# zzz5y/street_crafter

Measured on AMD Instinct MI355X. Metric: frames/sec @1M Gaussians 1920x1280 + PSNR vs ref; 1/2/4/8 MI355X, higher is better.
Workload: dtype f32

## Files before the change

### include/street_crafter_amd.h

```cpp
#ifndef STREET_CRAFTER_AMD_H
#define STREET_CRAFTER_AMD_H

#include <stddef.h>
#include <stdint.h>

#ifdef __cplusplus
extern "C" {
#endif

typedef void* sc_stream_t;

#define SC_OK 0
#define SC_EINVAL (-1)
#define SC_EWORKSPACE (-2)
#define SC_EUNSUPPORTED (-3)

const char* sc_version(void);
const char* sc_error_string(int code);
const char* sc_target_arch(void);
int sc_wait_i64(const int64_t* addr, int64_t value, int64_t timeout_us);

int sc_projection_fwd(const float* means, const float* quats, const float* scales,
                      const float* viewmats, const float* Ks, int C, int N, int width, int height,
                      float eps2d, float near_plane, float far_plane, float radius_clip,
// ... 33 lines not shown
                       const int32_t* tile_work ,
                       const float* viewmats ,
                       int32_t* view_registry ,
                       int32_t* tile_order ,
                       sc_stream_t stream);
int sc_view_slots(void);
int sc_view_registry_words(void);
int sc_isect_bin_bucket_capacity(void);
int sc_isect_split_limits(int64_t* out );
int64_t sc_isect_split_seg_bound(int64_t n_records, int nsb);
int sc_isect_split_bins(const uint64_t* keys, int64_t n, uint64_t lo, uint64_t hi, int32_t* bins);
int sc_isect_split_plan(const uint32_t* bin_counts, int cap, int32_t* range_of_bin, int32_t* n_ranges);
int sc_isect_bin_sort(const float* means2d, const int32_t* radii, const float* depths, int C, int N,
                      int tile_size, int tile_width, int tile_height,
                      const int32_t* isect_offsets, const int64_t* meta_dev,
                      void* count_workspace ,
                      int64_t capacity, int64_t rec_capacity, int64_t super_capacity,
                      int64_t* isect_ids , int32_t* flatten_ids,
                      void* workspace, size_t ws_bytes, sc_stream_t stream);
int sc_isect_ids_rebuild(const int32_t* flatten_ids, const int32_t* isect_offsets, const float* depths,
                         int C, int N, int tile_width, int tile_height, int64_t n_isects,
                         int64_t* isect_ids, sc_stream_t stream);
int sc_isect_bin_reset_cursors(void* count_workspace, int64_t CN, int C, int tile_width, int tile_height,
                               sc_stream_t stream);

int sc_isect_offsets(const int64_t* isect_ids, int64_t n_isects, int C, int tile_width,
                     int tile_height, int32_t* offsets, sc_stream_t stream);

int sc_sh_fwd(int degree, const float* dirs, const float* coeffs, const uint8_t* masks,
              int64_t M, int K, float* colors, sc_stream_t stream);
int sc_sh_bwd(int degree, const float* dirs, const float* coeffs, const uint8_t* masks,
              int64_t M, int K, const float* v_colors, float* v_coeffs, float* v_dirs,
              sc_stream_t stream);

int sc_rasterize_fwd(const float* means2d, const float* conics, const float* colors,
                     const float* opacities, const float* backgrounds, const uint8_t* tile_masks,
                     int C, int N, int D, int width, int height, int tile_size,
                     int tile_width, int tile_height,
                     const int32_t* isect_offsets, const int32_t* flatten_ids, int64_t n_isects,
                     float* render_colors, float* render_alphas,
                     int32_t* last_ids ,
                     const int32_t* tile_order ,
                     int32_t* tile_work ,
                     sc_stream_t stream);
int sc_tile_order_len(int total_tiles);
int sc_rasterize_bwd(const float* means2d, const float* conics, const float* colors,
                     const float* opacities, const float* backgrounds, const uint8_t* tile_masks,
                     int C, int N, int D, int width, int height, int tile_size,
                     int tile_width, int tile_height,
                     const int32_t* isect_offsets, const int32_t* flatten_ids, int64_t n_isects,
                     const float* render_alphas, const int32_t* last_ids,
                     const float* v_render_colors, const float* v_render_alphas,
                     float* v_means2d_abs, float* v_means2d, float* v_conics, float* v_colors,
                     float* v_opacities, const int32_t* tile_order ,
                     sc_stream_t stream);

size_t sc_knn_workspace_bytes(int64_t n);
int sc_knn3_mean_dist2(const float* points, int64_t n, float* out, void* workspace,
                       size_t ws_bytes, sc_stream_t stream);

int sc_point_project(const float* points, const float* colors, const float* opacities , float occ,
                     const float* radius_in , int N, const double* viewmat, double fx,
                     double fy, double cx, double cy, double focal_r, int width, int height, double near_plane,
                     double far_plane, int radius_mode, double scale, float knn_scale_down, int32_t* radii,
                     float* means2d, float* depths, float* records, sc_stream_t stream);
int sc_point_rasterize_fwd(const float* records, int N, int width, int height, int tile_width, int tile_height,
// ... 322 lines not shown
```

### street_crafter_amd/_lib.py

```python
from __future__ import annotations

import ctypes as C
import os

_HERE = os.path.dirname(os.path.abspath(__file__))
LIB_PATH = os.path.join(_HERE, "lib", "libstreet_crafter_hip.so")
DIAG_LIB_PATH = os.path.join(_HERE, "lib", "libstreet_crafter_hip_diag.so")

_lib = None
_path = LIB_PATH
_lock = __import__("threading").Lock()


def use_diagnostic_build(tag: str = ""):
    global _path
    want = DIAG_LIB_PATH.replace("_diag.so", f"_diag_{tag}.so") if tag else DIAG_LIB_PATH
    if _lib is not None and _path != want:
        raise RuntimeError("use_diagnostic_build() must be called before the library is first loaded")
    if not os.path.exists(want):
        raise ImportError(f"diagnostic library not built ({want} missing): "
                          "python -m street_crafter_amd.build --diag")
    _path = want

c_f32p = C.c_void_p
# ... 60 lines not shown
                                    c_f32p, c_f32p, c_f32p, c_stream]),
    "sc_projection_bwd": (C.c_int, [c_f32p, c_f32p, c_f32p, c_f32p, c_f32p, C.c_int, C.c_int, C.c_int,
                                    C.c_int, C.c_float, c_i32p, c_f32p, c_f32p, c_f32p, c_f32p, c_f32p,
                                    c_f32p, c_f32p, c_f32p, c_f32p, c_stream]),
    "sc_isect_workspace_bytes": (C.c_size_t, [C.c_int64]),
    "sc_isect_count": (C.c_int, [c_f32p, c_i32p, C.c_int, C.c_int, C.c_int, C.c_int, C.c_int, c_i32p,
                                 c_i64p, C.c_void_p, C.c_size_t, c_stream]),
    "sc_isect_emit": (C.c_int, [c_f32p, c_i32p, c_f32p, C.c_int, C.c_int, C.c_int, C.c_int, C.c_int,
                                c_i32p, C.c_int64, c_i64p, c_i32p, C.c_void_p, C.c_size_t, c_stream]),
    "sc_radix_sort_workspace_bytes": (C.c_size_t, [C.c_int64]),
    "sc_radix_sort_pairs_u64_i32": (C.c_int, [c_u64p, c_i32p, c_u64p, c_i32p, C.c_int64, C.c_int,
                                              C.c_void_p, C.c_size_t, c_stream]),
    "sc_isect_bin_workspace_bytes": (C.c_size_t, [C.c_int64, C.c_int, C.c_int, C.c_int, C.c_int64]),
    "sc_isect_bin_count": (C.c_int, [c_f32p, c_i32p, c_f32p, C.c_int, C.c_int, C.c_int, C.c_int, C.c_int, c_i32p,
                                     c_i32p, c_i64p, c_i64p, C.c_int64, C.c_void_p, C.c_size_t, c_i32p, c_f32p, c_i32p,
                                     c_i32p, c_stream]),
    "sc_view_slots": (C.c_int, []),
    "sc_view_registry_words": (C.c_int, []),
    "sc_isect_bin_bucket_capacity": (C.c_int, []),
    "sc_isect_split_limits": (C.c_int, [c_i64p]),
    "sc_isect_split_seg_bound": (C.c_int64, [C.c_int64, C.c_int]),
    "sc_isect_split_bins": (C.c_int, [c_u64p, C.c_int64, C.c_uint64, C.c_uint64, c_i32p]),
    "sc_isect_split_plan": (C.c_int, [C.c_void_p, C.c_int, c_i32p, c_i32p]),
    "sc_isect_bin_sort": (C.c_int, [c_f32p, c_i32p, c_f32p, C.c_int, C.c_int, C.c_int, C.c_int, C.c_int,
                                    c_i32p, c_i64p, C.c_void_p, C.c_int64, C.c_int64, C.c_int64, c_i64p,
                                    c_i32p, C.c_void_p, C.c_size_t, c_stream]),
    "sc_isect_ids_rebuild": (C.c_int, [c_i32p, c_i32p, c_f32p, C.c_int, C.c_int, C.c_int, C.c_int, C.c_int64, c_i64p,
                                       c_stream]),
    "sc_isect_bin_reset_cursors": (C.c_int, [C.c_void_p, C.c_int64, C.c_int, C.c_int, C.c_int, c_stream]),
    "sc_isect_offsets": (C.c_int, [c_i64p, C.c_int64, C.c_int, C.c_int, C.c_int, c_i32p, c_stream]),
    "sc_sh_fwd": (C.c_int, [C.c_int, c_f32p, c_f32p, c_u8p, C.c_int64, C.c_int, c_f32p, c_stream]),
    "sc_sh_bwd": (C.c_int, [C.c_int, c_f32p, c_f32p, c_u8p, C.c_int64, C.c_int, c_f32p, c_f32p, c_f32p,
                            c_stream]),
    "sc_rasterize_fwd": (C.c_int, [c_f32p, c_f32p, c_f32p, c_f32p, c_f32p, c_u8p, C.c_int, C.c_int, C.c_int,
                                   C.c_int, C.c_int, C.c_int, C.c_int, C.c_int, c_i32p, c_i32p, C.c_int64,
                                   c_f32p, c_f32p, c_i32p, c_i32p, c_i32p, c_stream]),
    "sc_rasterize_fwd_ed": (C.c_int, [c_f32p, c_f32p, c_f32p, c_f32p, c_f32p, c_u8p, C.c_int, C.c_int, C.c_int,
                                      C.c_int, C.c_int, C.c_int, C.c_int, C.c_int, c_i32p, c_i32p, C.c_int64,
                                      c_f32p, c_f32p, c_i32p, c_i32p, c_stream]),
    "sc_rasterize_fwd_planar": (C.c_int, [c_f32p, c_f32p, c_f32p, c_f32p, c_f32p, c_u8p, C.c_int, C.c_int, C.c_int,
                                          C.c_int, C.c_int, C.c_int, C.c_int, C.c_int, c_i32p, c_i32p, C.c_int64,
                                          c_f32p, c_f32p, c_i32p, c_i32p, c_stream]),
    "sc_group_extents": (C.c_int, [c_i32p, c_i32p, C.c_int64, c_u8p, C.c_int, C.c_int, C.c_int, C.c_int, C.c_int,
                                   c_i32p, c_stream]),
    "sc_rasterize_fwd_groups": (C.c_int, [c_f32p, c_f32p, c_f32p, c_f32p, c_u8p, c_i32p, C.c_int, C.c_int, C.c_int,
                                          C.c_int, C.c_int, C.c_int, C.c_int, C.c_int, C.c_int, c_i32p, c_i32p,
                                          C.c_int64, c_f32p, c_f32p, c_f32p, c_f32p, c_stream]),
    "sc_rasterize_fwd_groups_ids": (C.c_int, [c_f32p, c_f32p, c_f32p, c_f32p, c_u8p, c_i32p, C.c_int, C.c_int, C.c_int,
                                              C.c_int, C.c_int, C.c_int, C.c_int, C.c_int, C.c_int, c_i32p, c_i32p,
                                              C.c_int64, c_f32p, c_f32p, c_f32p, c_f32p, c_i32p, c_stream]),
    "sc_rasterize_bwd_groups": (C.c_int, [c_f32p, c_f32p, c_f32p, c_f32p, c_u8p, C.c_int, C.c_int, C.c_int, C.c_int,
                                          C.c_int, C.c_int, C.c_int, C.c_int, C.c_int, c_i32p, c_i32p, C.c_int64,
                                          c_f32p, c_f32p, c_i32p, c_f32p, c_f32p, c_f32p, c_f32p, c_f32p, c_f32p,
                                          c_f32p, c_f32p, c_f32p, c_stream]),
    "sc_camera_centers": (C.c_int, [c_f32p, C.c_int, c_f32p, c_stream]),
    "sc_projection_sh_fwd": (C.c_int, [c_f32p, c_f32p, c_f32p, c_f32p, c_f32p, c_f32p, c_f32p, c_f32p,
                                       C.c_int, C.c_int, C.c_int, C.c_int, C.c_int, C.c_int, C.c_float,
                                       C.c_float, C.c_float, C.c_float, C.c_int, c_i32p, c_f32p, c_f32p,
                                       c_f32p, c_f32p, c_f32p, c_f32p, c_stream]),
    "sc_projection_sh_bwd": (C.c_int, [c_f32p, c_f32p, c_f32p, c_f32p, c_f32p, c_f32p, c_f32p, c_f32p,
                                       C.c_int, C.c_int, C.c_int, C.c_int, C.c_int, C.c_int, C.c_float, C.c_int,
                                       c_i32p, c_f32p, c_f32p, c_f32p, c_f32p, c_f32p, c_f32p, c_f32p, c_f32p,
                                       c_f32p, c_f32p, c_f32p, c_stream]),
    "sc_rasterize_fwd_packed": (C.c_int, [c_f32p, c_f32p, c_u8p, C.c_int, C.c_int, C.c_int, C.c_int, C.c_int, C.c_int,
                                          c_i32p, c_i32p, C.c_int64, c_f32p, c_f32p, c_i32p, c_i32p, C.c_int, c_stream]),
    "sc_records_unpack": (C.c_int, [c_f32p, C.c_int64, c_f32p, c_f32p, c_f32p, c_stream]),
# ... 208 lines not shown
```

### street_crafter_amd/build.py

```python
from __future__ import annotations

import concurrent.futures as cf
import os
import subprocess
import sys

HERE = os.path.dirname(os.path.abspath(__file__))
CSRC = os.path.join(HERE, "csrc")
LIBDIR = os.path.join(HERE, "lib")
OBJDIR = os.path.join(HERE, "build")
LIB = os.path.join(LIBDIR, "libstreet_crafter_hip.so")
LIB_DIAG = os.path.join(LIBDIR, "libstreet_crafter_hip_diag.so")
BINDING = os.path.join(LIBDIR, "_sc_fast.so")
ARCH = "gfx950"

SOURCES = ["capi.hip", "projection.hip", "isect.hip", "isect_bin.hip", "radix_sort.hip", "sh.hip",
           "raster_fwd.hip", "raster_probe.hip", "raster_groups.hip", "raster_groups_bwd.hip", "raster_layers.hip", "raster_bwd.hip", "knn.hip", "fused_fwd.hip", "fused_bwd.hip", "point_raster.hip",
           "losses.hip", "regularizers.hip", "optim.hip", "densify.hip", "cubemap.hip", "lpips.hip", "resize.hip", "compose.hip",
           "frame_tail.hip", "point_assemble.hip", "frame_viz.hip"]
COMMON_FLAGS = ["-O3", f"--offload-arch={ARCH}", "-fPIC", "-std=c++17", "-Wall", "-Wno-unused-function",
                "-fno-gpu-rdc"]


def abi_hash() -> str:
    import hashlib
    with open(os.path.join(HERE, "..", "include", "street_crafter_amd.h"), "rb") as f:
        return hashlib.sha256(f.read()).hexdigest()[:16]


def _hipcc():
    for c in (os.environ.get("HIPCC"), "/opt/rocm/bin/hipcc", "hipcc"):
        if c and (os.path.isabs(c) and os.path.exists(c) or not os.path.isabs(c)):
            return c
    raise RuntimeError("hipcc not found")


def _deps(src):
    d = [os.path.join(CSRC, src)]
    d += [os.path.join(CSRC, f) for f in os.listdir(CSRC) if f.endswith(".h")]
    d.append(os.path.join(HERE, "..", "include", "street_crafter_amd.h"))
    return d


def _stale(target, deps):
    if not os.path.exists(target):
        return True
    t = os.path.getmtime(target)
    return any(os.path.getmtime(d) > t for d in deps)


def _compile(src, force, verbose, diag=False):
    tag = os.environ.get("SC_DIAG_TAG", "") if diag else ""
# ... 67 lines not shown
```

### street_crafter_amd/csrc/sh.hip

```cpp
#include "sh_common.h"

#pragma clang fp contract(off)

namespace {

template <int DEG>
__global__ __launch_bounds__(256) void sh_fwd_kernel(const float* __restrict__ dirs,
                                                     const float* __restrict__ coeffs,
                                                     const uint8_t* __restrict__ masks, int64_t M,
                                                     int K, float* __restrict__ colors) {
    const int64_t i = (int64_t)blockIdx.x * 256 + threadIdx.x;
    if (i >= M) return;
    float r = 0.f, g = 0.f, b = 0.f;
    if (!masks || masks[i])
        sh_eval<DEG>(dirs[i * 3 + 0], dirs[i * 3 + 1], dirs[i * 3 + 2], coeffs + i * (int64_t)K * 3, r, g, b);
    colors[i * 3 + 0] = r; colors[i * 3 + 1] = g; colors[i * 3 + 2] = b;
}

}

#pragma clang fp contract(fast)

namespace {

template <int DEG, bool VEC>
__global__ __launch_bounds__(256) void sh_bwd_kernel(const float* __restrict__ dirs,
                                                     const float* __restrict__ coeffs,
                                                     const uint8_t* __restrict__ masks, int64_t M,
                                                     int K, const float* __restrict__ v_colors,
                                                     float* __restrict__ v_coeffs,
                                                     float* __restrict__ v_dirs) {
    constexpr int NB = (DEG + 1) * (DEG + 1);
    constexpr int NV = (NB * 3 + 3) / 4;
    const int64_t i = (int64_t)blockIdx.x * 256 + threadIdx.x;
    if (i >= M) return;
    float* vc = v_coeffs + i * (int64_t)K * 3;
    const bool on = !masks || masks[i];
    float vdx = 0.f, vdy = 0.f, vdz = 0.f;
    if (on) {
        const float dx = dirs[i * 3 + 0], dy = dirs[i * 3 + 1], dz = dirs[i * 3 + 2];
        float Y[NB];
        sh_basis<DEG>(dx, dy, dz, Y);
        const float vr = v_colors[i * 3 + 0], vg = v_colors[i * 3 + 1], vb = v_colors[i * 3 + 2];
        if (VEC) {
            float o[NV * 4];
#pragma unroll
            for (int f = 0; f < NV * 4; ++f) o[f] = (f < NB * 3) ? Y[f / 3] * ((f % 3) == 0 ? vr : ((f % 3) == 1 ? vg : vb)) : 0.f;
// ... 24 lines not shown
                w[k] = VEC ? vr * cf[k * 3 + 0] + vg * cf[k * 3 + 1] + vb * cf[k * 3 + 2]
                           : vr * c[k * 3 + 0] + vg * c[k * 3 + 1] + vb * c[k * 3 + 2];
            sh_dir_vjp<DEG>(dx, dy, dz, w, vdx, vdy, vdz);
        }
    } else if (VEC) {
        for (int j = 0; j < (K * 3) / 4; ++j) reinterpret_cast<float4*>(vc)[j] = make_float4(0.f, 0.f, 0.f, 0.f);
    } else {
        for (int k = 0; k < K; ++k) { vc[k * 3 + 0] = 0.f; vc[k * 3 + 1] = 0.f; vc[k * 3 + 2] = 0.f; }
    }
    if (v_dirs) { v_dirs[i * 3 + 0] = vdx; v_dirs[i * 3 + 1] = vdy; v_dirs[i * 3 + 2] = vdz; }
}

}

extern "C" int sc_sh_fwd(int degree, const float* dirs, const float* coeffs, const uint8_t* masks,
                         int64_t M, int K, float* colors, sc_stream_t stream) {
    if (degree < 0 || degree > 4 || M < 0 || K < (degree + 1) * (degree + 1)) return SC_EINVAL;
    if (M == 0) return SC_OK;
    if (!dirs || !coeffs || !colors) return SC_EINVAL;
    const int64_t nb = (M + 255) / 256;
    if (nb > 0x7fffffff) return SC_EINVAL;
    dim3 grid((unsigned)nb), block(256);
    switch (degree) {
        case 0: hipLaunchKernelGGL(sh_fwd_kernel<0>, grid, block, 0, sc_s(stream), dirs, coeffs, masks, M, K, colors); break;
        case 1: hipLaunchKernelGGL(sh_fwd_kernel<1>, grid, block, 0, sc_s(stream), dirs, coeffs, masks, M, K, colors); break;
        case 2: hipLaunchKernelGGL(sh_fwd_kernel<2>, grid, block, 0, sc_s(stream), dirs, coeffs, masks, M, K, colors); break;
        case 3: hipLaunchKernelGGL(sh_fwd_kernel<3>, grid, block, 0, sc_s(stream), dirs, coeffs, masks, M, K, colors); break;
        default: hipLaunchKernelGGL(sh_fwd_kernel<4>, grid, block, 0, sc_s(stream), dirs, coeffs, masks, M, K, colors); break;
    }
    SC_LAUNCH_CHECK();
    return SC_OK;
}

extern "C" int sc_sh_bwd(int degree, const float* dirs, const float* coeffs, const uint8_t* masks,
                         int64_t M, int K, const float* v_colors, float* v_coeffs, float* v_dirs,
                         sc_stream_t stream) {
    if (degree < 0 || degree > 4 || M < 0 || K < (degree + 1) * (degree + 1)) return SC_EINVAL;
    if (M == 0) return SC_OK;
    if (!dirs || !coeffs || !v_colors || !v_coeffs) return SC_EINVAL;
    const int64_t nb = (M + 255) / 256;
    if (nb > 0x7fffffff) return SC_EINVAL;
    dim3 grid((unsigned)nb), block(256);
    const bool vec = (K * 3) % 4 == 0 && ((uintptr_t)coeffs % 16) == 0 && ((uintptr_t)v_coeffs % 16) == 0;
#define SC_SH_BWD(D)                                                                                              \
    if (vec) hipLaunchKernelGGL((sh_bwd_kernel<D, true>), grid, block, 0, sc_s(stream), dirs, coeffs, masks, M, K, \
                                v_colors, v_coeffs, v_dirs);                                                       \
    else hipLaunchKernelGGL((sh_bwd_kernel<D, false>), grid, block, 0, sc_s(stream), dirs, coeffs, masks, M, K,     \
                            v_colors, v_coeffs, v_dirs)
    switch (degree) {
        case 0: SC_SH_BWD(0); break;
        case 1: SC_SH_BWD(1); break;
        case 2: SC_SH_BWD(2); break;
        case 3: SC_SH_BWD(3); break;
        default: SC_SH_BWD(4); break;
    }
#undef SC_SH_BWD
    SC_LAUNCH_CHECK();
    return SC_OK;
}
```

### street_crafter_amd/dist.py

```python
from __future__ import annotations

import os
import socket
import subprocess
import sys
import time
from typing import Callable, Dict, List, Optional, Sequence

import torch
import torch.distributed as dist

from . import _lib

ROUNDING = {"video": 0, "save_image": 1}


def frames_for_rank(n_frames: int, rank: int, world: int) -> List[int]:
    return list(range(rank, n_frames, world))


def _hwc_view(x: torch.Tensor):
    if x.dim() != 3 or x.shape[0] != 3:
        return None
    s0, s1, s2 = x.stride()
    if s0 == 1 and s2 >= 3 and s1 == x.shape[2] * s2:
        return x, s2, 1
    if s2 == 1 and s1 == x.shape[2] and s0 >= x.shape[1] * x.shape[2]:
        return x, 1, s0
    return None


_STREAM_FN = []


def _raw_stream(t: torch.Tensor):
    if not _STREAM_FN:
        from .rendering import _stream
        _STREAM_FN.append(_stream)
    return _STREAM_FN[0](t)


def to_uint8_frame(rgb_chw: torch.Tensor, acc: Optional[torch.Tensor] = None,
                   sky_rgb_chw: Optional[torch.Tensor] = None, rounding: str = "video",
                   out: Optional[torch.Tensor] = None) -> torch.Tensor:
    if rounding not in ROUNDING:
        raise ValueError(f"rounding must be one of {sorted(ROUNDING)}, got {rounding!r}")
    if (acc is None) != (sky_rgb_chw is None):
        raise ValueError("acc and sky_rgb_chw go together (two-pass frame) or are both None")
    x = rgb_chw.detach() if rgb_chw.requires_grad else rgb_chw
    H, W = x.shape[1], x.shape[2]
    if out is None:
        out = torch.empty((H, W, 3), dtype=torch.uint8, device=x.device)
    else:
        assert out.shape == (H, W, 3) and out.dtype == torch.uint8 and out.is_contiguous() and out.device == x.device
    if x.is_cuda and x.dtype == torch.float32:
        fg = _hwc_view(x)
        sky = _hwc_view(sky_rgb_chw.detach()) if sky_rgb_chw is not None else None
        a = acc.detach().reshape(H, W) if acc is not None else None
        if fg is not None and (sky_rgb_chw is None or (sky is not None and a.is_contiguous()
                                                      and a.dtype == torch.float32)):
            b = _lib.binding()
            if fg[2] != 1 or fg[1] < 3 or (sky is not None and (sky[2] != 1 or sky[1] < 3)):
                rc = b.frame_composite_u8_strided(fg[0].data_ptr(), fg[1], fg[2], 0 if a is None else a.data_ptr(),
                                                  0 if sky is None else sky[0].data_ptr(), 1 if sky is None else sky[1],
                                                  1 if sky is None else sky[2], H * W, ROUNDING[rounding], out,
                                                  _raw_stream(x))
            else:
                rc = b.frame_composite_u8(fg[0].data_ptr(), fg[1], 0 if a is None else a.data_ptr(),
                                          0 if sky is None else sky[0].data_ptr(), 0 if sky is None else sky[1],
                                          H * W, ROUNDING[rounding], out, _raw_stream(x))
            if rc:
                _lib.check(rc, "sc_frame_composite_u8")
            return out
    v = x.float().clamp(0.0, 1.0)
    if sky_rgb_chw is not None:
        v = (v + sky_rgb_chw.detach().float().clamp(0.0, 1.0) * (1.0 - acc.detach().float().reshape(1, H, W))).clamp(0.0, 1.0)
    v = v * 255.0
    if ROUNDING[rounding]:
        v = v + 0.5
    out.copy_(v.to(torch.uint8).permute(1, 2, 0))
    return out
# ... 373 lines not shown
```

### street_crafter_amd/isect.py

```python
from __future__ import annotations

import collections
import math
import os
import threading
import weakref
from typing import Optional, Tuple

import torch
from torch import Tensor

from . import _lib
from .lazy import LazyTensor as _LazyTensor


def _env_on(name: str, default: bool = True) -> bool:
    v = os.environ.get(name)
    return default if v is None or v == "" else v not in ("0", "false", "False", "off", "no")


class _Switches:
    __slots__ = ("tile_order", "lazy_ids", "view_slots", "packed_records", "defer_isect", "planar_out", "fused_train")

    def __init__(self):
        self.tile_order = _env_on("SC_TILE_ORDER")
        self.lazy_ids = _env_on("SC_LAZY_IDS")
        self.view_slots = _env_on("SC_VIEW_SLOTS")
        self.packed_records = _env_on("SC_PACKED_RECORDS")
        self.defer_isect = _env_on("SC_DEFER_ISECT")
        self.planar_out = _env_on("SC_PLANAR_OUTPUT")
        self.fused_train = _env_on("SC_FUSED_TRAIN", False)

    def flip(self, name: str, value: bool) -> bool:
        prev = getattr(self, name)
        setattr(self, name, bool(value))
        return prev


def _predicted_capacities(history, bucket_cap) -> Tuple[int, int, int]:
    mi, mr, ms = map(max, zip(*history))
    ms_pred = ms + ms // 8 + 64
    if ms <= bucket_cap < ms_pred:
        ms_pred = bucket_cap
    return mi + mi // 8 + 4096, mr + mr // 8 + 4096, ms_pred


class _OperatorState:
    KEYS_MAX = 64

    def __init__(self):
        self.prediction, self.history, self.last_meta = {}, {}, {}
        self.history_len = 8
        self.tile_work, self.view_registry = {}, {}
        self.stats = {"calls": 0, "speculative_ok": 0, "exact_relaunch": 0}
        self.bucket_cap = {}
        self.sched_sizes = {}

    def tables(self):
        return (("predictions", self.prediction), ("history", self.history), ("last_meta", self.last_meta),
                ("tile_work", self.tile_work), ("view_registry", self.view_registry))

    def reset(self, idx=None) -> dict:
        dropped = {}
        for name, table in self.tables():
            keys = [k for k in table if idx is None or (k[0] if isinstance(k, tuple) else k) == idx]
            for k in keys:
                table.pop(k, None)
            dropped[name] = len(keys)
        return dropped

    def record(self, key, sizes, bucket_cap):
        hist = self.history.get(key)
        if hist is None:
            hist = self.history[key] = collections.deque(maxlen=self.history_len)
            while len(self.history) > self.KEYS_MAX:
                old = next(iter(self.history))
                for table in (self.history, self.prediction, self.last_meta):
                    table.pop(old, None)
        hist.append(sizes)
        self.last_meta[key] = sizes
        self.prediction[key] = _predicted_capacities(hist, bucket_cap)


_SWITCH = _Switches()
_STATE = _OperatorState()

_ISECT_MODE = {"mode": "bin"}
# ... 2 lines not shown
def set_isect_mode(mode: str) -> str:
    assert mode in ("bin", "radix")
    prev = _ISECT_MODE["mode"]
    _ISECT_MODE["mode"] = mode
    return prev


def set_lazy_isect_ids(enabled: bool) -> bool:
    return _SWITCH.flip("lazy_ids", enabled)


def set_deferred_isect(enabled: bool) -> bool:
    return _SWITCH.flip("defer_isect", enabled)


def _p(t: Optional[Tensor]):
    return None if t is None else t.data_ptr()


_RAW_STREAM = getattr(torch._C, "_cuda_getCurrentRawStream", None)


def _stream(t: Tensor):
    if _RAW_STREAM is not None:
        return _RAW_STREAM(t.device.index if t.device.index is not None else torch.cuda.current_device())
    return torch.cuda.current_stream(t.device).cuda_stream


def _req(t: Tensor, name: str, dtype=torch.float32):
    if type(t) is Tensor and t.dtype is dtype and t.is_cuda and t.is_contiguous():
        return t
    if not isinstance(t, Tensor):
        raise TypeError(f"{name} must be a torch.Tensor, got {type(t)}")
    if not t.is_cuda:
        raise RuntimeError(f"{name} must live on a HIP device (got {t.device}); "
                           "street_crafter_amd has no CPU path")
    if t.dtype != dtype:
        raise TypeError(f"{name} must be {dtype}, got {t.dtype}")
    return t.contiguous()


def _ws(nbytes: int, device) -> Tensor:
    return torch.empty(max(int(nbytes), 256), dtype=torch.uint8, device=device)


_WARNED = set()


def _warn_once(key, msg, *args):
    if key not in _WARNED:
        _WARNED.add(key)
        import logging
        logging.getLogger("street_crafter_amd").warning(msg, *args)


@torch.no_grad()
def isect_tiles(means2d: Tensor, radii: Tensor, depths: Tensor, tile_size: int, tile_width: int,
                tile_height: int, sort: bool = True, packed: bool = False,
                n_cameras: Optional[int] = None, camera_ids: Optional[Tensor] = None,
                gaussian_ids: Optional[Tensor] = None) -> Tuple[Tensor, Tensor, Tensor]:
    if packed:
        raise NotImplementedError("packed=True is not supported (reference passes packed=False)")
    view_cams = getattr(means2d, "_sc_viewmats", None)
    means2d = _req(means2d.detach() if means2d.requires_grad else means2d, "means2d")
    radii = _req(radii, "radii", torch.int32)
    depths = _req(depths.detach() if depths.requires_grad else depths, "depths")
# ... 284 lines not shown
```

### street_crafter_amd/rendering.py

```python
from __future__ import annotations

import math
from typing import Optional, Tuple

import torch
from torch import Tensor

from . import _lib
from .lazy import LazyTensor as _LazyTensor
from .isect import (_ISECT_MODE, _PINNED_META, _RAW_STREAM, _STATE, _SWITCH, _BinCall, _MetaSlot,
                    _OperatorState, _PendingIsect, _Switches, _bin_launch_ran, _check_isect_count, _isect_tiles_bin,
                    _isect_tiles_radix, _p, _req, _stream, _tile_work, _view_registry, _warn_once, _ws,
                    isect_offset_encode, isect_tiles, set_deferred_isect, set_isect_mode, set_lazy_isect_ids)

__all__ = ["fully_fused_projection", "isect_tiles", "isect_offset_encode", "spherical_harmonics",
           "rasterize_to_pixels", "rasterization"]


class _NoGradCtx:
    needs_input_grad = (False,) * 16

    def save_for_backward(self, *tensors):
        pass

    def mark_non_differentiable(self, *tensors):
        pass

    def __setattr__(self, name, value):
        pass


_NO_GRAD_CTX = _NoGradCtx()
_EMPTY = {}


def _needs_grad(*args) -> bool:
    return torch.is_grad_enabled() and any(isinstance(a, Tensor) and a.requires_grad for a in args)


def _call(fn, *args):
    if _needs_grad(*args):
# ... 90 lines not shown
                           scales: Optional[Tensor], viewmats: Tensor, Ks: Tensor, width: int,
                           height: int, eps2d: float = 0.3, near_plane: float = 0.01,
                           far_plane: float = 1e10, radius_clip: float = 0.0, packed: bool = False,
                           sparse_grad: bool = False, calc_compensations: bool = False):
    if covars is not None:
        raise NotImplementedError("covars= is not supported: the reference passes quats/scales "
                                  "(street_gaussian_renderer.py:219-224)")
    if packed:
        raise NotImplementedError("packed=True is not supported: the reference passes packed=False "
                                  "(street_gaussian_renderer.py:228)")
    assert quats is not None and scales is not None, "quats and scales are required"
    means = _req(means, "means")
    quats = _req(quats, "quats")
    scales = _req(scales, "scales")
    viewmats = _req(viewmats, "viewmats")
    Ks = _req(Ks, "Ks")
    N = means.shape[0]
    C = viewmats.shape[0]
    assert means.shape == (N, 3), means.shape
    assert quats.shape == (N, 4), quats.shape
    assert scales.shape == (N, 3), scales.shape
    assert viewmats.shape == (C, 4, 4), viewmats.shape
    assert Ks.shape == (C, 3, 3), Ks.shape
    nat = _native() if _needs_grad(means, quats, scales) else None
    if nat is not None:
        out = nat.projection_autograd(means, quats, scales, viewmats, Ks, int(width), int(height), float(eps2d),
                                      float(near_plane), float(far_plane), float(radius_clip), bool(calc_compensations),
                                      _RAW_STREAM)
    else:
        out = _call(_Projection, means, quats, scales, viewmats, Ks, width, height, eps2d, near_plane,
                                far_plane, radius_clip, calc_compensations)
    if N and C:
        out[1]._sc_viewmats = viewmats
    if calc_compensations:
        return out
    return (*out, None)


def set_tile_order(enabled: bool) -> bool:
    return _SWITCH.flip("tile_order", enabled)


def set_packed_records(enabled: bool) -> bool:
    return _SWITCH.flip("packed_records", enabled)


def set_view_slots(enabled: bool) -> bool:
    return _SWITCH.flip("view_slots", enabled)


class _SphericalHarmonics(torch.autograd.Function):
    @staticmethod
    def forward(ctx, degree, dirs, coeffs, masks):
        rc, colors = _lib.binding().sh_fwd(int(degree), dirs, coeffs, masks, _stream(dirs))
        if rc:
            _lib.check(rc, "sc_sh_fwd")
        ctx.save_for_backward(dirs, coeffs, masks if masks is not None else torch.empty(0, device=dirs.device))
        ctx.meta = (int(degree), masks is not None)
        return colors

    @staticmethod
    def backward(ctx, v_colors):
        dirs, coeffs, masks = ctx.saved_tensors
        degree, has_mask = ctx.meta
        v_colors = v_colors.contiguous()
        with _probe("spherical_harmonics_bwd"):
            rc, v_coeffs, v_dirs = _lib.binding().sh_bwd(degree, dirs, coeffs, masks if has_mask else None, v_colors,
                                                         bool(ctx.needs_input_grad[1]), _stream(dirs))
        if rc:
            _lib.check(rc, "sc_sh_bwd")
        return None, v_dirs, (v_coeffs if ctx.needs_input_grad[2] else None), None


def spherical_harmonics(degrees_to_use: int, dirs: Tensor, coeffs: Tensor,
                        masks: Optional[Tensor] = None) -> Tensor:
    assert 0 <= degrees_to_use <= 4, degrees_to_use
    assert (degrees_to_use + 1) ** 2 <= coeffs.shape[-2], coeffs.shape
    assert dirs.shape[:-1] == coeffs.shape[:-2], (dirs.shape, coeffs.shape)
    assert dirs.shape[-1] == 3 and coeffs.shape[-1] == 3, (dirs.shape, coeffs.shape)
    dirs = _req(dirs, "dirs")
    coeffs = _req(coeffs, "coeffs")
    if masks is not None:
        assert masks.shape == dirs.shape[:-1], masks.shape
        if not masks.is_cuda:
            raise RuntimeError("masks must live on a HIP device")
        if masks.dtype == torch.bool:
            masks = masks.contiguous().view(torch.uint8)
        elif masks.dtype != torch.uint8:
            masks = masks.to(torch.uint8).contiguous()
        else:
            masks = masks.contiguous()
    nat = _native() if _needs_grad(dirs, coeffs) else None
    if nat is not None:
        return nat.sh_autograd(int(degrees_to_use), dirs, coeffs, masks, _RAW_STREAM)
    return _call(_SphericalHarmonics, int(degrees_to_use), dirs, coeffs, masks)


def set_planar_output(enabled: bool) -> bool:
    return _SWITCH.flip("planar_out", enabled)


_RASTER_SIDE = {}


def set_raster_side_stream(device, side, main=None):
    idx = device if isinstance(device, int) else torch.device(device).index
    if idx is None:
        idx = torch.cuda.current_device()
    tab = _RASTER_SIDE.setdefault(idx, {})
    key = None if main is None else int(main.cuda_stream)
    prev = tab.get(key)
    if side is None:
        tab.pop(key, None)
        if not tab:
            _RASTER_SIDE.pop(idx, None)
    else:
        tab[key] = side
    return prev


def reset_state(device=None) -> dict:
    idx = None if device is None else (device if isinstance(device, int) else torch.device(device).index)
    for d, slot in getattr(_PINNED_META, "slots", {}).items():
        if idx is None or d == idx:
            slot.settle_pending("settle_reset", "reset_state: settling a never observed isect_tiles call failed (%s: %s)")
    return _STATE.reset(idx)


# ... 104 lines not shown
    conics = _req(conics, "conics")
    colors = _req(colors, "colors")
    opacities = _req(opacities, "opacities")
    isect_offsets = _req(isect_offsets, "isect_offsets", torch.int32)
    if type(flatten_ids) is _LazyTensor:
        flatten_ids = flatten_ids.plain()
    flatten_ids = _req(flatten_ids, "flatten_ids", torch.int32)
    C, N = opacities.shape
    D = colors.shape[-1]
    assert means2d_c.shape == (C, N, 2), means2d_c.shape
    assert conics.shape == (C, N, 3), conics.shape
    assert colors.shape == (C, N, D), colors.shape
    assert isect_offsets.ndim == 3 and isect_offsets.shape[0] == C, isect_offsets.shape
    th, tw = isect_offsets.shape[1], isect_offsets.shape[2]
    assert tw * tile_size >= image_width, "image_width must fit in tile_width * tile_size"
    assert th * tile_size >= image_height, "image_height must fit in tile_height * tile_size"
    if not 1 <= D <= 32:
        raise NotImplementedError(f"colour channels must be in 1..32, got {D}")
    if backgrounds is not None:
        backgrounds = _req(backgrounds, "backgrounds")
        assert backgrounds.shape == (C, D), backgrounds.shape
    if masks is not None:
        assert masks.shape == isect_offsets.shape, masks.shape
        if not masks.is_cuda:
            raise RuntimeError("masks must live on a HIP device")
        masks = masks.to(torch.uint8).contiguous()

    nat = _native() if _needs_grad(means2d_c, conics, colors, opacities, backgrounds) else None
    if nat is not None:
        order, work = _sched_of(isect_offsets, C * tw * th)
        return nat.rasterize_autograd(means2d_c, conics, colors, opacities, backgrounds, masks, int(image_width),
                                      int(image_height), int(tile_size), isect_offsets, flatten_ids, bool(absgrad), order,
                                      work, caller_means2d, _RAW_STREAM)
    return _call(_Rasterize, means2d_c, conics, colors, opacities, backgrounds, masks, int(image_width),
                            int(image_height), int(tile_size), isect_offsets, flatten_ids, bool(absgrad),
                            _AbsgradTarget(caller_means2d))


def camera_centers(viewmats: Tensor) -> Tensor:
    lib = _lib.load()
    viewmats = _req(viewmats, "viewmats")
    out = torch.empty((viewmats.shape[0], 3), dtype=torch.float32, device=viewmats.device)
    _lib.check(lib.sc_camera_centers(_p(viewmats), viewmats.shape[0], _p(out), _stream(viewmats)),
               "sc_camera_centers")
    return out


_FUSED_RASTERIZATION = True


def set_fused_rasterization(enabled: bool) -> bool:
    global _FUSED_RASTERIZATION
    prev, _FUSED_RASTERIZATION = _FUSED_RASTERIZATION, bool(enabled)
    return prev


def _fused_forward_ok(tensors, sh_degree, render_mode, tile_size, colors) -> bool:
    if not _FUSED_RASTERIZATION or sh_degree is None or render_mode not in ("RGB+D", "RGB+ED"):
        return False
    if tile_size != 16 or colors.dim() != 3 or colors.shape[-1] != 3:
        return False
    if torch.is_grad_enabled() and any(t is not None and t.requires_grad for t in tensors):
        return False
    return True


def set_fused_training(enabled: bool) -> bool:
    return _SWITCH.flip("fused_train", enabled)

# ... 276 lines not shown
```

Measured before the change: 3127.

## Add deferred glue tensors fusing torch elementwise ops into custom kernels

Introduces tensor subclasses that record simple elementwise torch ops (gt, add, clamp, div, cat, views) on renderer outputs during inference without running them. Recognised patterns are replaced by dedicated kernels: SH evaluation masked directly by radii, a fused add+clamp_min+cat into a packed colour/depth float4 buffer, and skipping a clamp before uint8 frame conversion. The goal is fewer small kernel launches and less intermediate memory traffic in the per-frame glue, at the cost of substantial Python dispatch overhead and complexity around materialisation and version tracking.

```diff
diff --git a/include/street_crafter_amd.h b/include/street_crafter_amd.h
--- a/include/street_crafter_amd.h
+++ b/include/street_crafter_amd.h
@@ -89,6 +89,10 @@
 int sc_sh_bwd(int degree, const float* dirs, const float* coeffs, const uint8_t* masks,
               int64_t M, int K, const float* v_colors, float* v_coeffs, float* v_dirs,
               sc_stream_t stream);
+int sc_sh_fwd_radii(int degree, const float* dirs, const float* coeffs, const int32_t* radii,
+                    int64_t M, int K, float* colors, sc_stream_t stream);
+int sc_pack_colors_depth(const float* colors, const float* depths, int64_t M, float add, float floor,
+                         float* out, sc_stream_t stream);
 
 int sc_rasterize_fwd(const float* means2d, const float* conics, const float* colors,
                      const float* opacities, const float* backgrounds, const uint8_t* tile_masks,
diff --git a/street_crafter_amd/_lib.py b/street_crafter_amd/_lib.py
--- a/street_crafter_amd/_lib.py
+++ b/street_crafter_amd/_lib.py
@@ -116,6 +116,8 @@
     "sc_sh_fwd": (C.c_int, [C.c_int, c_f32p, c_f32p, c_u8p, C.c_int64, C.c_int, c_f32p, c_stream]),
     "sc_sh_bwd": (C.c_int, [C.c_int, c_f32p, c_f32p, c_u8p, C.c_int64, C.c_int, c_f32p, c_f32p, c_f32p,
                             c_stream]),
+    "sc_sh_fwd_radii": (C.c_int, [C.c_int, c_f32p, c_f32p, c_i32p, C.c_int64, C.c_int, c_f32p, c_stream]),
+    "sc_pack_colors_depth": (C.c_int, [c_f32p, c_f32p, C.c_int64, C.c_float, C.c_float, c_f32p, c_stream]),
     "sc_rasterize_fwd": (C.c_int, [c_f32p, c_f32p, c_f32p, c_f32p, c_f32p, c_u8p, C.c_int, C.c_int, C.c_int,
                                    C.c_int, C.c_int, C.c_int, C.c_int, C.c_int, c_i32p, c_i32p, C.c_int64,
                                    c_f32p, c_f32p, c_i32p, c_i32p, c_i32p, c_stream]),
diff --git a/street_crafter_amd/build.py b/street_crafter_amd/build.py
--- a/street_crafter_amd/build.py
+++ b/street_crafter_amd/build.py
@@ -17,7 +17,7 @@
 SOURCES = ["capi.hip", "projection.hip", "isect.hip", "isect_bin.hip", "radix_sort.hip", "sh.hip",
            "raster_fwd.hip", "raster_probe.hip", "raster_groups.hip", "raster_groups_bwd.hip", "raster_layers.hip", "raster_bwd.hip", "knn.hip", "fused_fwd.hip", "fused_bwd.hip", "point_raster.hip",
            "losses.hip", "regularizers.hip", "optim.hip", "densify.hip", "cubemap.hip", "lpips.hip", "resize.hip", "compose.hip",
-           "frame_tail.hip", "point_assemble.hip", "frame_viz.hip"]
+           "frame_tail.hip", "point_assemble.hip", "frame_viz.hip", "glue.hip"]
 COMMON_FLAGS = ["-O3", f"--offload-arch={ARCH}", "-fPIC", "-std=c++17", "-Wall", "-Wno-unused-function",
                 "-fno-gpu-rdc"]
 
diff --git a/street_crafter_amd/csrc/glue.hip b/street_crafter_amd/csrc/glue.hip
--- /dev/null
+++ b/street_crafter_amd/csrc/glue.hip
@@ -0,0 +1,34 @@
+#include "sc_common.h"
+
+#pragma clang fp contract(off)
+
+namespace {
+
+__device__ __forceinline__ float clamp_min_like_torch(float v, float floor) { return (v != v) ? v : fmaxf(v, floor); }
+
+__global__ __launch_bounds__(256) void pack_colors_depth_kernel(const float* __restrict__ colors,
+                                                                const float* __restrict__ depths, int64_t M, float add,
+                                                                float floor, float4* __restrict__ out) {
+    const int64_t i = (int64_t)blockIdx.x * 256 + threadIdx.x;
+    if (i >= M) return;
+    const float r = colors[i * 3 + 0] + add, g = colors[i * 3 + 1] + add, b = colors[i * 3 + 2] + add;
+    out[i] = make_float4(clamp_min_like_torch(r, floor), clamp_min_like_torch(g, floor), clamp_min_like_torch(b, floor),
+                         depths[i]);
+}
+
+}
+
+extern "C" int sc_pack_colors_depth(const float* colors, const float* depths, int64_t M, float add, float floor,
+                                    float* out, sc_stream_t stream) {
+    if (M < 0) return SC_EINVAL;
+    if (M == 0) return SC_OK;
+    if (!colors || !depths || !out || ((uintptr_t)out % 16) != 0 || ((uintptr_t)colors % 4) != 0 ||
+        ((uintptr_t)depths % 4) != 0)
+        return SC_EINVAL;
+    const int64_t nb = (M + 255) / 256;
+    if (nb > 0x7fffffff) return SC_EINVAL;
+    hipLaunchKernelGGL(pack_colors_depth_kernel, dim3((unsigned)nb), dim3(256), 0, sc_s(stream), colors, depths, M, add,
+                       floor, reinterpret_cast<float4*>(out));
+    SC_LAUNCH_CHECK();
+    return SC_OK;
+}
diff --git a/street_crafter_amd/csrc/sh.hip b/street_crafter_amd/csrc/sh.hip
--- a/street_crafter_amd/csrc/sh.hip
+++ b/street_crafter_amd/csrc/sh.hip
@@ -13,6 +13,19 @@
     if (i >= M) return;
     float r = 0.f, g = 0.f, b = 0.f;
     if (!masks || masks[i])
+        sh_eval<DEG>(dirs[i * 3 + 0], dirs[i * 3 + 1], dirs[i * 3 + 2], coeffs + i * (int64_t)K * 3, r, g, b);
+    colors[i * 3 + 0] = r; colors[i * 3 + 1] = g; colors[i * 3 + 2] = b;
+}
+
+template <int DEG>
+__global__ __launch_bounds__(256) void sh_fwd_radii_kernel(const float* __restrict__ dirs,
+                                                           const float* __restrict__ coeffs,
+                                                           const int32_t* __restrict__ radii, int64_t M,
+                                                           int K, float* __restrict__ colors) {
+    const int64_t i = (int64_t)blockIdx.x * 256 + threadIdx.x;
+    if (i >= M) return;
+    float r = 0.f, g = 0.f, b = 0.f;
+    if (radii[i] > 0)
         sh_eval<DEG>(dirs[i * 3 + 0], dirs[i * 3 + 1], dirs[i * 3 + 2], coeffs + i * (int64_t)K * 3, r, g, b);
     colors[i * 3 + 0] = r; colors[i * 3 + 1] = g; colors[i * 3 + 2] = b;
 }
@@ -103,6 +116,25 @@
     return SC_OK;
 }
 
+extern "C" int sc_sh_fwd_radii(int degree, const float* dirs, const float* coeffs, const int32_t* radii,
+                               int64_t M, int K, float* colors, sc_stream_t stream) {
+    if (degree < 0 || degree > 4 || M < 0 || K < (degree + 1) * (degree + 1)) return SC_EINVAL;
+    if (M == 0) return SC_OK;
+    if (!dirs || !coeffs || !radii || !colors) return SC_EINVAL;
+    const int64_t nb = (M + 255) / 256;
+    if (nb > 0x7fffffff) return SC_EINVAL;
+    dim3 grid((unsigned)nb), block(256);
+    switch (degree) {
+        case 0: hipLaunchKernelGGL(sh_fwd_radii_kernel<0>, grid, block, 0, sc_s(stream), dirs, coeffs, radii, M, K, colors); break;
+        case 1: hipLaunchKernelGGL(sh_fwd_radii_kernel<1>, grid, block, 0, sc_s(stream), dirs, coeffs, radii, M, K, colors); break;
+        case 2: hipLaunchKernelGGL(sh_fwd_radii_kernel<2>, grid, block, 0, sc_s(stream), dirs, coeffs, radii, M, K, colors); break;
+        case 3: hipLaunchKernelGGL(sh_fwd_radii_kernel<3>, grid, block, 0, sc_s(stream), dirs, coeffs, radii, M, K, colors); break;
+        default: hipLaunchKernelGGL(sh_fwd_radii_kernel<4>, grid, block, 0, sc_s(stream), dirs, coeffs, radii, M, K, colors); break;
+    }
+    SC_LAUNCH_CHECK();
+    return SC_OK;
+}
+
 extern "C" int sc_sh_bwd(int degree, const float* dirs, const float* coeffs, const uint8_t* masks,
                          int64_t M, int K, const float* v_colors, float* v_coeffs, float* v_dirs,
                          sc_stream_t stream) {
diff --git a/street_crafter_amd/deferred.py b/street_crafter_amd/deferred.py
--- /dev/null
+++ b/street_crafter_amd/deferred.py
@@ -0,0 +1,373 @@
+from __future__ import annotations
+
+import math
+import weakref
+
+import torch
+
+from .isect import _STATE, _SWITCH, _stream
+from .lazy import LazyTensor, _is_metadata, _is_shape_free
+
+_T = torch.Tensor
+_NOSUB = torch._C.DisableTorchFunctionSubclass
+_F32, _I32 = torch.float32, torch.int32
+
+
+def set_deferred_glue(enabled: bool, min_gaussians: int = None) -> bool:
+    if min_gaussians is not None:
+        _SWITCH.defer_glue_min = int(min_gaussians)
+    return _SWITCH.flip("defer_glue", enabled)
+
+
+def tag(t, n_gaussians: int = None):
+    if (type(t) is _T and _SWITCH.defer_glue and not torch.is_grad_enabled()
+            and (n_gaussians is None or n_gaussians >= _SWITCH.defer_glue_min)):
+        return GlueTensor(t)
+    return t
+
+
+def plain(t):
+    if type(t) is GlueTensor:
+        return t.__dict__["_sc_plain"]
+    if type(t) is DeferredTensor:
+        t.materialize()
+        return t.__dict__["_sc_plain"]
+    return t
+
+
+def _roots_of(t):
+    d = t.__dict__
+    if type(t) is GlueTensor:
+        return (t if d["_sc_root"] is None else d["_sc_root"],)
+    return d["_sc_roots"]
+
+
+def _settle_dependants(t):
+    for root in _roots_of(t):
+        for x in [w() for w in root.__dict__["_sc_deps"]]:
+            if x is not None:
+                x.materialize()
+
+
+def _has_dependants(t) -> bool:
+    for root in _roots_of(t):
+        for w in root.__dict__["_sc_deps"]:
+            x = w()
+            if x is not None and x.__dict__.get("_sc_fill") is not None:
+                return True
+    return False
+
+
+class GlueTensor(torch.Tensor):
+
+    @staticmethod
+    def __new__(cls, data: torch.Tensor, root=None):
+        t = _T._make_subclass(cls, data, False)
+        d = t.__dict__
+        d["_sc_plain"] = data
+        d["_sc_root"] = root
+        if root is None:
+            d["_sc_deps"] = []
+        return t
+
+    def plain(self) -> torch.Tensor:
+        return self.__dict__["_sc_plain"]
+
+    def __deepcopy__(self, memo):
+        out = self.__dict__["_sc_plain"].clone()
+        memo[id(self)] = out
+        return out
+
+    def __reduce_ex__(self, proto):
+        return self.__dict__["_sc_plain"].__reduce_ex__(proto)
+
+    @classmethod
+    def __torch_function__(cls, func, types, args=(), kwargs=None):
+        return _glue_function(func, types, args, kwargs or {})
+
+
+class DeferredTensor(LazyTensor):
+
+    @staticmethod
+    def __new__(cls, buffer, fill, kind, srcs, params, roots):
+        t = _T._make_subclass(cls, buffer, False)
+        t.__dict__.update(_sc_fill=fill, _sc_resolve=None, _sc_plain=buffer, _sc_kind=kind, _sc_srcs=srcs,
+                          _sc_params=params, _sc_roots=roots,
+                          _sc_versions=tuple([s.__dict__["_sc_plain"]._version for s in srcs]))
+        ref = weakref.ref(t)
+        for r in roots:
+            deps = r.__dict__["_sc_deps"]
+            if len(deps) >= 16:
+                deps[:] = [w for w in deps if w() is not None and w().__dict__.get("_sc_fill") is not None]
+            deps.append(ref)
+        return t
+
+    @property
+    def pending(self) -> bool:
+        return self.__dict__.get("_sc_fill") is not None
+
+    @classmethod
+    def __torch_function__(cls, func, types, args=(), kwargs=None):
+        return _glue_function(func, types, args, kwargs or {})
+
+
+def _operand(s):
+    if type(s) is DeferredTensor:
+        s.materialize()
+    return s.__dict__["_sc_plain"]
+
+
+def _fill_op(self):
+    d = self.__dict__
+    fn, params, kwargs = d["_sc_params"]
+    fn(*[_operand(s) for s in d["_sc_srcs"]], *params, **kwargs, out=d["_sc_plain"])
+    _STATE.glue_stats["torch_filled"] += 1
+    d["_sc_srcs"] = ()
+
+
+def _fill_view(self):
+    d = self.__dict__
+    d["_sc_srcs"][0].materialize()
+    d["_sc_srcs"] = ()
+
+
+_LAYOUT = {}
+
+
+def _layout(fn, plains, params, kwargs):
+    p = plains[0]
+    if len(plains) == 1 and not kwargs:
+        key = (fn, p.shape, p.stride(), p.dtype, type(params[0]))
+    else:
+        key = (fn, tuple([(p.shape, p.stride(), p.dtype) for p in plains]), tuple([type(v) for v in params]),
+               tuple([k for k, v in kwargs.items() if v is not None]))
+    got = _LAYOUT.get(key)
+    if got is None:
+        if len(_LAYOUT) > 256:
+            _LAYOUT.clear()
+        metas = [torch.empty_strided(p.shape, p.stride(), dtype=p.dtype, device="meta") for p in plains]
+        m = fn(*metas, *params, **kwargs)
+        got = _LAYOUT[key] = (tuple(m.shape), tuple(m.stride()), m.dtype)
+    return got
+
+
+def _defer(fn, srcs, params, kwargs):
+    plains = [s.__dict__["_sc_plain"] for s in srcs]
+    shape, stride, dtype = _layout(fn, plains, params, kwargs)
+    buf = torch.empty_strided(shape, stride, dtype=dtype, device=plains[0].device)
+    roots = _roots_of(srcs[0])
+    for s in srcs[1:]:
+        roots = roots + tuple(r for r in _roots_of(s) if all(r is not q for q in roots))
+    _STATE.glue_stats["deferred"] += 1
+    return DeferredTensor(buf, _fill_op, fn.__name__, tuple(srcs), (fn, params, kwargs), roots)
+
+
+def _view(func, x, rest):
+    v = func(x.__dict__["_sc_plain"], *rest)
+    return DeferredTensor(v, _fill_view, "view", (x,), (func, rest), x.__dict__["_sc_roots"])
+
+
+def _tagged(t, *dtypes) -> bool:
+    return type(t) is GlueTensor and t.__dict__["_sc_plain"].dtype in dtypes
+
+
+def _pending(t, kind=None) -> bool:
+    if type(t) is not DeferredTensor:
+        return False
+    d = t.__dict__
+    return d.get("_sc_fill") is not None and (kind is None or d["_sc_kind"] == kind)
+
+
+def _basic_index(idx) -> bool:
+    if type(idx) is int:
+        return True
+    if type(idx) is tuple:
+        for i in idx:
+            if not (i is Ellipsis or i is None or type(i) is int or type(i) is slice):
+                return False
+        return True
+    return idx is None or idx is Ellipsis or type(idx) is slice
+
+
+def _rule_gt(func, args, kwargs):
+    if len(args) == 2 and not kwargs and _tagged(args[0], _I32, _F32) and type(args[1]) in (int, float):
+        return _defer(torch.gt, (args[0],), (args[1],), {})
+    return None
+
+
+def _rule_add(func, args, kwargs):
+    if len(args) == 2 and not kwargs and _tagged(args[0], _F32) and type(args[1]) is float:
+        return _defer(torch.add, (args[0],), (args[1],), {})
+    return None
+
+
+def _rule_clamp_min(func, args, kwargs):
+    if len(args) == 2 and not kwargs and _pending(args[0], "add") and type(args[1]) is float:
+        return _defer(torch.clamp_min, (args[0],), (args[1],), {})
+    return None
+
+
+def _rule_clamp(func, args, kwargs):
+    if not args or len(args) > 3 or not _tagged(args[0], _F32) or any(k not in ("min", "max") for k in kwargs):
+        return None
+    lo = args[1] if len(args) > 1 else kwargs.get("min")
+    hi = args[2] if len(args) > 2 else kwargs.get("max")
+    if (len(args) > 1 and "min" in kwargs) or (len(args) > 2 and "max" in kwargs):
+        return None
+    if (lo is None and hi is None) or any(v is not None and type(v) is not float for v in (lo, hi)):
+        return None
+    return _defer(torch.clamp, (args[0],), (), {"min": lo, "max": hi})
+
+
+def _rule_div(func, args, kwargs):
+    if len(args) != 2 or kwargs:
+        return None
+    a, b = args
+    if _tagged(a, _I32, _F32) and type(b) is float:
+        return _defer(torch.div, (a,), (b,), {})
+    if _tagged(a, _F32) and _pending(b, "clamp"):
+        return _defer(torch.div, (a, b), (), {})
+    return None
+
+
+def _rule_getitem(func, args, kwargs):
+    if len(args) != 2 or kwargs or not _basic_index(args[1]):
+        return None
+    x = args[0]
+    if type(x) is GlueTensor:
+        d = x.__dict__
+        return GlueTensor(func(d["_sc_plain"], args[1]), x if d["_sc_root"] is None else d["_sc_root"])
+    if _pending(x):
+        return _view(func, x, (args[1],))
+    return None
+
+
+def _rule_view(func, args, kwargs):
+    if kwargs or not args or not _pending(args[0]):
+        return None
+    rest = args[1:]
+    if not all(type(v) is int or (type(v) in (tuple, list) and all(type(i) is int for i in v)) for v in rest):
+        return None
+    return _view(func, args[0], rest)
+
+
+def _finite32(v: float) -> bool:
+    return math.isfinite(v) and abs(v) < 3.0e38
+
+
+def _unmoved(x) -> bool:
+    d = x.__dict__
+    return all(s.__dict__["_sc_plain"]._version == v for s, v in zip(d["_sc_srcs"], d["_sc_versions"]))
+
+
+def _rule_cat(func, args, kwargs):
+    if not args or any(k != "dim" for k in kwargs) or len(args) > 2 or (len(args) == 2 and kwargs):
+        return None
+    seq = args[0]
+    dim = args[1] if len(args) == 2 else kwargs.get("dim", 0)
+    if type(seq) not in (tuple, list) or len(seq) != 2 or type(dim) is not int or dim not in (-1, 2):
+        return None
+    cm, dep = seq
+    if not _pending(cm, "clamp_min") or not _unmoved(cm):
+        return None
+    ad = cm.__dict__["_sc_srcs"][0]
+    if not _pending(ad, "add") or not _unmoved(ad):
+        return None
+    col = ad.__dict__["_sc_srcs"][0]
+    if type(col) is not GlueTensor or col.__dict__["_sc_root"] is not None:
+        return None
+    cp = col.__dict__["_sc_plain"]
+    dp = dep.__dict__["_sc_plain"] if type(dep) is GlueTensor else dep
+    a, b = ad.__dict__["_sc_params"][1][0], cm.__dict__["_sc_params"][1][0]
+    if (type(dp) is not _T or not cp.is_cuda or cp.dim() != 3 or cp.shape[2] != 3 or not cp.is_contiguous()
+            or dp.dtype is not _F32 or dp.device != cp.device or dp.requires_grad or not _finite32(a) or not _finite32(b)):
+        return None
+    C, N = cp.shape[0], cp.shape[1]
+    if tuple(dp.shape) != (C, N, 1) or (N > 1 and dp.stride(1) != 1) or (C > 1 and N > 0 and dp.stride(0) != N):
+        return None
+    from . import _lib
+    out = torch.empty((C, N, 4), dtype=_F32, device=cp.device)
+    _lib.check(_lib.load().sc_pack_colors_depth(cp.data_ptr(), dp.data_ptr(), C * N, a, b, out.data_ptr(), _stream(cp)),
+               "sc_pack_colors_depth")
+    _STATE.glue_stats["fused"] += 3
+    return out
+
+
+_RULES = {"gt": _rule_gt, "add": _rule_add, "clamp_min": _rule_clamp_min, "clamp": _rule_clamp, "div": _rule_div,
+          "__getitem__": _rule_getitem, "permute": _rule_view, "select": _rule_view, "unsqueeze": _rule_view,
+          "cat": _rule_cat}
+
+
+def _flat(args, kwargs):
+    for a in args:
+        if isinstance(a, (list, tuple)):
+            yield from a
+        else:
+            yield a
+    yield from kwargs.values()
+
+
+def _glue_function(func, types, args, kwargs):
+    name = getattr(func, "__name__", "")
+    rule = _RULES.get(name)
+    if rule is not None and _SWITCH.defer_glue and not torch.is_grad_enabled():
+        out = rule(func, args, kwargs)
+        if out is not None:
+            return out
+    if _is_shape_free(func) or _is_metadata(func):
+        return LazyTensor.__torch_function__(func, types, args, kwargs)
+    mine = [a for a in _flat(args, kwargs) if type(a) in (GlueTensor, DeferredTensor) and _has_dependants(a)]
+    if mine and ("out" in kwargs or name == "__setitem__" or (name.endswith("_") and not name.endswith("__"))):
+        for a in mine:
+            _settle_dependants(a)
+        mine = []
+    out = LazyTensor.__torch_function__(func, types, args, kwargs)
+    first = args[0] if args else None
+    if type(out) is GlueTensor and out is not first:
+        with _NOSUB():
+            out = out.as_subclass(_T)
+    elif type(out) in (tuple, list) and any(type(o) in (GlueTensor, DeferredTensor) for o in out):
+        with _NOSUB():
+            out = type(out)(o.as_subclass(_T) if type(o) in (GlueTensor, DeferredTensor) else o for o in out)
+    if mine:
+        with _NOSUB():
+            outs = [o for o in (out if type(out) in (tuple, list) else (out,)) if isinstance(o, _T)]
+            for a in mine:
+                base = a.__dict__["_sc_plain"].untyped_storage().data_ptr()
+                if any(o.untyped_storage().data_ptr() == base for o in outs):
+                    _settle_dependants(a)
+    return out
+
+
+def radii_of_mask(masks):
+    if not _pending(masks, "gt") or not _unmoved(masks):
+        return None
+    d = masks.__dict__
+    thr = d["_sc_params"][1][0]
+    src = d["_sc_srcs"][0]
+    p = src.__dict__["_sc_plain"]
+    if thr != 0 or p.dtype is not _I32 or not p.is_cuda or not p.is_contiguous():
+        return None
+    return p
+
+
+def clamp01_source(x):
+    ops = []
+    while _pending(x, "view"):
+        d = x.__dict__
+        ops.append(d["_sc_params"])
+        x = d["_sc_srcs"][0]
+    if not _pending(x, "clamp") or not _unmoved(x):
+        return None
+    d = x.__dict__
+    kw = d["_sc_params"][2]
+    if kw["min"] != 0.0 or kw["max"] != 1.0:
+        return None
+    p = d["_sc_srcs"][0].__dict__["_sc_plain"]
+    for func, rest in reversed(ops):
+        p = func(p, *rest)
+    return p
+
+
+def count_fused(n: int = 1):
+    _STATE.glue_stats["fused"] += n
diff --git a/street_crafter_amd/dist.py b/street_crafter_amd/dist.py
--- a/street_crafter_amd/dist.py
+++ b/street_crafter_amd/dist.py
@@ -40,6 +40,22 @@
     return _STREAM_FN[0](t)
 
 
+_GLUE = []
+
+
+def _unclamped(img):
+    if type(img) is not torch.Tensor and img is not None:
+        if not _GLUE:
+            from . import deferred
+            _GLUE.append(deferred)
+        if type(img) is _GLUE[0].DeferredTensor:
+            src = _GLUE[0].clamp01_source(img)
+            if src is not None:
+                _GLUE[0].count_fused()
+                return src
+    return img
+
+
 def to_uint8_frame(rgb_chw: torch.Tensor, acc: Optional[torch.Tensor] = None,
                    sky_rgb_chw: Optional[torch.Tensor] = None, rounding: str = "video",
                    out: Optional[torch.Tensor] = None) -> torch.Tensor:
@@ -47,6 +63,7 @@
         raise ValueError(f"rounding must be one of {sorted(ROUNDING)}, got {rounding!r}")
     if (acc is None) != (sky_rgb_chw is None):
         raise ValueError("acc and sky_rgb_chw go together (two-pass frame) or are both None")
+    rgb_chw, sky_rgb_chw = _unclamped(rgb_chw), _unclamped(sky_rgb_chw)
     x = rgb_chw.detach() if rgb_chw.requires_grad else rgb_chw
     H, W = x.shape[1], x.shape[2]
     if out is None:
diff --git a/street_crafter_amd/isect.py b/street_crafter_amd/isect.py
--- a/street_crafter_amd/isect.py
+++ b/street_crafter_amd/isect.py
@@ -20,7 +20,8 @@
 
 
 class _Switches:
-    __slots__ = ("tile_order", "lazy_ids", "view_slots", "packed_records", "defer_isect", "planar_out", "fused_train")
+    __slots__ = ("tile_order", "lazy_ids", "view_slots", "packed_records", "defer_isect", "planar_out", "fused_train",
+                 "defer_glue", "defer_glue_min")
 
     def __init__(self):
         self.tile_order = _env_on("SC_TILE_ORDER")
@@ -30,6 +31,8 @@
         self.defer_isect = _env_on("SC_DEFER_ISECT")
         self.planar_out = _env_on("SC_PLANAR_OUTPUT")
         self.fused_train = _env_on("SC_FUSED_TRAIN", False)
+        self.defer_glue = _env_on("SC_DEFER_GLUE")
+        self.defer_glue_min = int(os.environ.get("SC_DEFER_GLUE_MIN") or 262144)
 
     def flip(self, name: str, value: bool) -> bool:
         prev = getattr(self, name)
@@ -53,6 +56,7 @@
         self.history_len = 8
         self.tile_work, self.view_registry = {}, {}
         self.stats = {"calls": 0, "speculative_ok": 0, "exact_relaunch": 0}
+        self.glue_stats = {"deferred": 0, "fused": 0, "torch_filled": 0}
         self.bucket_cap = {}
         self.sched_sizes = {}
 
@@ -121,6 +125,11 @@
         return t
     if not isinstance(t, Tensor):
         raise TypeError(f"{name} must be a torch.Tensor, got {type(t)}")
+    p = t.__dict__.get("_sc_plain")
+    if p is not None:
+        if isinstance(t, _LazyTensor):
+            t.materialize()
+        return _req(p, name, dtype)
     if not t.is_cuda:
         raise RuntimeError(f"{name} must live on a HIP device (got {t.device}); "
                            "street_crafter_amd has no CPU path")
diff --git a/street_crafter_amd/rendering.py b/street_crafter_amd/rendering.py
--- a/street_crafter_amd/rendering.py
+++ b/street_crafter_amd/rendering.py
@@ -7,6 +7,8 @@
 from torch import Tensor
 
 from . import _lib
+from . import deferred as _glue
+from .deferred import set_deferred_glue
 from .lazy import LazyTensor as _LazyTensor
 from .isect import (_ISECT_MODE, _PINNED_META, _RAW_STREAM, _STATE, _SWITCH, _BinCall, _MetaSlot,
                     _OperatorState, _PendingIsect, _Switches, _bin_launch_ran, _check_isect_count, _isect_tiles_bin,
@@ -163,6 +165,8 @@
                                 far_plane, radius_clip, calc_compensations)
     if N and C:
         out[1]._sc_viewmats = viewmats
+    if nat is None and _SWITCH.defer_glue and not torch.is_grad_enabled():
+        out = (_glue.tag(out[0], C * N), *out[1:])
     if calc_compensations:
         return out
     return (*out, None)
@@ -211,6 +215,14 @@
     assert dirs.shape[-1] == 3 and coeffs.shape[-1] == 3, (dirs.shape, coeffs.shape)
     dirs = _req(dirs, "dirs")
     coeffs = _req(coeffs, "coeffs")
+    if type(masks) is _glue.DeferredTensor and not torch.is_grad_enabled():
+        radii = _glue.radii_of_mask(masks)
+        if radii is not None and radii.shape == dirs.shape[:-1] and radii.device == dirs.device:
+            colors = torch.empty(dirs.shape, dtype=torch.float32, device=dirs.device)
+            _lib.check(_lib.load().sc_sh_fwd_radii(int(degrees_to_use), _p(dirs), _p(coeffs), _p(radii), radii.numel(),
+                                                   coeffs.shape[-2], _p(colors), _stream(dirs)), "sc_sh_fwd_radii")
+            _glue.count_fused()
+            return _glue.tag(colors, radii.numel())
     if masks is not None:
         assert masks.shape == dirs.shape[:-1], masks.shape
         if not masks.is_cuda:
@@ -224,7 +236,7 @@
     nat = _native() if _needs_grad(dirs, coeffs) else None
     if nat is not None:
         return nat.sh_autograd(int(degrees_to_use), dirs, coeffs, masks, _RAW_STREAM)
-    return _call(_SphericalHarmonics, int(degrees_to_use), dirs, coeffs, masks)
+    return _glue.tag(_call(_SphericalHarmonics, int(degrees_to_use), dirs, coeffs, masks), dirs.numel() // 3)
 
 
 def set_planar_output(enabled: bool) -> bool:
@@ -395,9 +407,10 @@
         return nat.rasterize_autograd(means2d_c, conics, colors, opacities, backgrounds, masks, int(image_width),
                                       int(image_height), int(tile_size), isect_offsets, flatten_ids, bool(absgrad), order,
                                       work, caller_means2d, _RAW_STREAM)
-    return _call(_Rasterize, means2d_c, conics, colors, opacities, backgrounds, masks, int(image_width),
-                            int(image_height), int(tile_size), isect_offsets, flatten_ids, bool(absgrad),
-                            _AbsgradTarget(caller_means2d))
+    render_colors, render_alphas = _call(_Rasterize, means2d_c, conics, colors, opacities, backgrounds, masks,
+                                         int(image_width), int(image_height), int(tile_size), isect_offsets, flatten_ids,
+                                         bool(absgrad), _AbsgradTarget(caller_means2d))
+    return _glue.tag(render_colors, C * N), _glue.tag(render_alphas, C * N)
 
 
 def camera_centers(viewmats: Tensor) -> Tensor:
```

Result: slower. 3057 (-2.2%).
